# nuggy875/NeRF_pytorch_paeng

Measured on AMD Instinct MI355X. Metric: rays/sec (4096-ray batch, 64c+128f samples) + 800×800 frame render ms, higher is better.
Workload: dtype f32

## Files before the change

### nerf_pytorch_paeng_amd/csrc/api.hip

```cpp
#include <string>
#include "half_layout.h"

namespace minerf {

ABI_ERROR_STATE(, MI_NERF_EHIP)

int device_cus() {
    static std::atomic<int> cus[MN_MAX_DEVICES] = {};
    int dev = 0;
    if (hipGetDevice(&dev) != hipSuccess) return 256;
    std::atomic<int>& slot = cus[dev & (MN_MAX_DEVICES - 1)];
    int c = slot.load(std::memory_order_relaxed);
    if (c <= 0) {
        hipDeviceProp_t prop;
        c = (hipGetDeviceProperties(&prop, dev) == hipSuccess && prop.multiProcessorCount > 0) ? prop.multiProcessorCount : 256;
        slot.store(c, std::memory_order_relaxed);
    }
    return c;
}
int ensure_lds_opt_in(LdsOptIn& state, const void* kernel) {
    int dev = 0;
    MN_HIP(hipGetDevice(&dev));
    std::atomic<bool>& done = state.done[dev & (MN_MAX_DEVICES - 1)];
    if (!done.load(std::memory_order_acquire)) {
        MN_HIP(hipFuncSetAttribute(kernel, hipFuncAttributeMaxDynamicSharedMemorySize, 160 * 1024));
        done.store(true, std::memory_order_release);
    }
    return MI_NERF_OK;
}

int mlp_rays_fp32(const mi_nerf_net*, const void*, const float*, const float*, int64_t, int, float*, hipStream_t);
int mlp_embedded_fp32(const mi_nerf_net*, const void*, const float*, int64_t, float*, hipStream_t);
int mlp_rays_bf16(const mi_nerf_net*, const void*, const float*, const float*, int64_t, int, float*, hipStream_t, int points_per_wave, const StratDraw* strat,
                  FineDraw* fine = nullptr);
int mlp_rays_f16(const mi_nerf_net*, const void*, const float*, const float*, int64_t, int, float*, hipStream_t, int points_per_wave, const StratDraw* strat,
                 FineDraw* fine);
int mlp_rays_f16s(const mi_nerf_net*, const void*, const float*, const float*, int64_t, int, float*, hipStream_t);
int mlp_rays_f16s_stash(const mi_nerf_net*, const void*, const float*, const float*, int64_t, int, float*, float*, float*, float*, unsigned*, unsigned*,
                        hipStream_t);
int wgrad_products(int, const float* const*, const int*, const int*, const float* const*, const int*, const int*, int64_t, float* const*, const int*,
                   float* const*, void*, size_t, hipStream_t, bool);
int mlp_rays_fp32_stash(const mi_nerf_net*, const void*, const float*, const float*, int64_t, int, float*, float*, float*, float*, unsigned*,
                        unsigned*, hipStream_t);
int mlp_backward_fp32(const mi_nerf_net*, const void*, const void*, const float*, const float*, int64_t, int, const float*, const void*, void*,
                      size_t, float*, int, hipStream_t, const float*, int64_t, int);
int mlp_embedded_fp32_stash(const mi_nerf_net*, const void*, const float*, int64_t, float*, float*, float*, float*, unsigned*, unsigned*,
                            hipStream_t);
int train_layout(const mi_nerf_net*, int64_t, int, mi_nerf_train_layout*);
size_t wgrad_scratch_bytes();
int pack_apply(const int32_t*, const float*, size_t, void*, hipStream_t);
int frames_image_metrics(const float*, const float*, int64_t, float*, void*, size_t, hipStream_t);
int frames_nanmax(const float*, int64_t, float*, void*, size_t, hipStream_t);
int frames_to8b(const float*, int64_t, const float*, unsigned char*, hipStream_t);
int frames_rays_rgb(int, int, const float*, const float*, const float*, int64_t, float*, hipStream_t);
// ... 326 lines not shown
    return frames_rays_rgb(W, H, k4, poses, images, n_img, out, (hipStream_t)st);
}
int mi_nerf_permute_rows(const float* src, const int64_t* perm, int64_t n, int row_floats, float* dst, void* st) {
    return frames_permute_rows(src, perm, n, row_floats, dst, (hipStream_t)st);
}

size_t mi_nerf_render_workspace_bytes(const mi_nerf_render_cfg* cfg, int64_t n_rays) {
    mi_nerf_workspace_layout L;
    if (workspace_layout(cfg, n_rays, &L)) return 0;
    return L.total;
}
int mi_nerf_render_workspace_layout(const mi_nerf_render_cfg* cfg, int64_t n_rays, mi_nerf_workspace_layout* out) {
    return workspace_layout(cfg, n_rays, out);
}

int mi_nerf_render_rays(const mi_nerf_net* net, const void* packed_c, const void* packed_f, const mi_nerf_render_cfg* cfg,
                        const float* rays, int64_t n, const float* t_rand, const float* u, void* ws, size_t ws_bytes,
                        float* rgb_c, float* disp_c, float* rgb_f, float* disp_f, void* stream) {
    hipStream_t st = (hipStream_t)stream;
    mi_nerf_workspace_layout L;
    if (int rc = workspace_layout(cfg, n, &L)) return rc;
    if (n == 0) return MI_NERF_OK;
    MN_CHECK_ARG(ws_bytes >= L.total, "workspace too small: %zu < %zu", ws_bytes, L.total);
    MN_CHECK_ARG(rays && rgb_c && disp_c && packed_c && (ws || L.total == 0), "NULL pointer");
    MN_CHECK_ARG(cfg->Nf == 0 || (packed_f && rgb_f && disp_f), "fine pass needs packed_fine and outputs");
    MN_CHECK_ARG(cfg->reserved == 0, "mi_nerf_render_cfg.reserved must be 0");
    char* w = (char*)ws;
    float* z_c = (float*)(w + L.z_c);
    float* raw_c = (float*)(w + L.raw_c);
    float* wts_c = (float*)(w + L.weights_c);
    const int Sc = cfg->Sc, St = cfg->Sc + cfg->Nf;
    ModePlan p;
    if (int rc = mode_plan(cfg->mode, &p)) return rc;
    if (p.coarse == Family::F16 || p.fine == Family::F16)
        if (int rc = check_net_half(net, "f16")) return rc;
    if (p.coarse == Family::F16S || p.fine == Family::F16S)
        if (int rc = check_net_f16s_forward(net)) return rc;
    FineDraw fd{};
    if (p.coarse == Family::BF16 || p.coarse == Family::F16) {
        const StratDraw sd{cfg->near_, cfg->far_, t_rand, cfg->seed, cfg->ray_offset, z_c};
        if (cfg->Nf > 0) fd = FineDraw{cfg->Nf, cfg->det, u, cfg->seed, cfg->ray_offset, rgb_c, disp_c, wts_c, (float*)(w + L.z_f), false};
        if (int rc = mlp_rays_family(p.coarse, net, packed_c, rays, nullptr, n, Sc, raw_c, st, p.points_per_wave, &sd,
                                     cfg->Nf > 0 && p.points_per_wave == 0 ? &fd : nullptr))
            return rc;
    } else {
        if (int rc = stage_stratified(n, Sc, cfg->near_, cfg->far_, t_rand, cfg->seed, cfg->ray_offset, z_c, st)) return rc;
        if (int rc = mlp_rays_family(p.coarse, net, packed_c, rays, z_c, n, Sc, raw_c, st, p.points_per_wave)) return rc;
    }
    if (cfg->Nf == 0) return stage_composite(raw_c, z_c, rays, 6, n, Sc, rgb_c, disp_c, nullptr, wts_c, nullptr, st);
    {
        float* z_f = (float*)(w + L.z_f);
        float* raw_f = (float*)(w + L.raw_f);
        if (!fd.taken)
            if (int rc = stage_composite_fine_z(raw_c, z_c, rays, n, Sc, cfg->Nf, cfg->det, u, cfg->seed, cfg->ray_offset, rgb_c, disp_c, wts_c, z_f, st))
                return rc;
        if (int rc = mlp_rays_family(p.fine, net, packed_f, rays, z_f, n, St, raw_f, st, p.points_per_wave)) return rc;
        if (int rc = stage_composite(raw_f, z_f, rays, 6, n, St, rgb_f, disp_f, nullptr, nullptr, nullptr, st)) return rc;
    }
    return MI_NERF_OK;
}

int mi_nerf_time_mlp_rays(const mi_nerf_net* net, const void* packed, const float* rays, const float* z, int64_t n_rays, int S,
                          float* raw, int iters, int mode, float* avg_ms, void* stream) {
    hipStream_t st = (hipStream_t)stream;
    MN_CHECK_ARG(iters >= 1 && avg_ms, "bad iters / NULL output");
    ModePlan p;
    if (int rc = mode_plan(mode, &p)) return rc;
    MN_CHECK_ARG(p.coarse == p.fine, "MI_NERF_MODE_* %d is two kernel families (mi_nerf_render_rays only): one network, one kernel family", mode);
    if (p.fine == Family::F16)
        if (int rc = check_net_half(net, "f16")) return rc;
// ... 86 lines not shown
```

### nerf_pytorch_paeng_amd/csrc/layout.h

```cpp
#pragma once
#include <stdint.h>
#include <stddef.h>

namespace minerf {

constexpr int QUAD_BYTES = 1024;
constexpr int SLOT_QUADS = 16;
constexpr int SLOT_BYTES = QUAD_BYTES * SLOT_QUADS;
constexpr int HEADER_BYTES = 1024;
constexpr uint32_t BLOB_MAGIC = 0x4D494E46u;

__host__ __device__ constexpr int pe_ksteps(int L) { return ((3 * L + 2 + 3) / 4) * 4; }

constexpr int KERNEL_LX = 10, KERNEL_LD = 4;

constexpr int MAX_KERNEL_WIDTH = 512;
__host__ __device__ constexpr int kernel_width(int W) { return W <= 128 ? 128 : (W <= 256 ? 256 : (W <= 384 ? 384 : 512)); }
__host__ __device__ constexpr bool wide_kernel_width(int Wk) { return Wk > 256; }
__host__ __device__ constexpr int pe_ksteps16(int L) { return (((3 * L + 1) / 2 + 1 + 3) / 4) * 4; }
__host__ __device__ constexpr bool native_width(int W) { return W == 128 || W == 256; }

struct BlobLayout {
    uint32_t stream_off;
    uint32_t stream_bytes_hoist;
// ... 24 lines not shown
    uint32_t quads = pe_quads;
    for (int l = 1; l < D; ++l) quads += h_quads + ((skip >= 0 && l == skip + 1) ? pe_quads : 0);
    quads += h_quads;
    quads += (uint32_t)(W / 2 / 4) * (NT / 2);
    b.stream_off = HEADER_BYTES;
    b.stream_bytes_hoist = round_up_u32(quads, SLOT_QUADS) * QUAD_BYTES;
    uint32_t full = round_up_u32(quads, SLOT_QUADS) + round_up_u32((uint32_t)(pe_ksteps(L_d) / 4) * (NT / 2), SLOT_QUADS);
    b.stream_bytes_full = full * QUAD_BYTES;
    b.side_off = b.stream_off + b.stream_bytes_full;
    uint32_t f = 0;
    b.bias_trunk = f; f += (uint32_t)D * W;
    b.bias_feat = f;  f += W;
    b.bias_d = f;     f += W / 2;
    b.dens_w = f;     f += W;
    b.dens_b = f;     f += 4;
    b.color_w = f;    f += 3 * (W / 2);
    b.color_b = f;    f += 4;
    b.wdir_t = f;     f += (uint32_t)in_d * (W / 2);
    b.side_floats = round_up_u32(f, 4);
    b.total_bytes = b.side_off + b.side_floats * 4;
    return b;
}

struct SideTables {
    const char* stream;
    const float* side;
    int D;
    int skip_layer;
    unsigned stream_bytes;
    unsigned side_floats;
    unsigned o_bias_trunk, o_bias_feat, o_bias_d, o_wdir_t;
    unsigned o_dens_w, o_dens_b, o_color_w, o_color_b;
    unsigned o_head_b;
};
inline int skip_layer_of(int D, int skip) { return (skip >= 0 && skip + 1 < D) ? skip + 1 : -1; }

inline SideTables side_tables(const BlobLayout& L, const void* packed_dev, int D, int skip, bool full_stream) {
    SideTables t{};
    t.stream = (const char*)packed_dev + L.stream_off;
    t.side = (const float*)((const char*)packed_dev + L.side_off);
    t.D = D;
    t.skip_layer = skip_layer_of(D, skip);
    t.stream_bytes = full_stream ? L.stream_bytes_full : L.stream_bytes_hoist;
    t.side_floats = L.side_floats;
    t.o_bias_trunk = L.bias_trunk; t.o_bias_feat = L.bias_feat; t.o_bias_d = L.bias_d; t.o_wdir_t = L.wdir_t;
    t.o_dens_w = L.dens_w; t.o_dens_b = L.dens_b; t.o_color_w = L.color_w; t.o_color_b = L.color_b;
// ... 39 lines not shown
```

### nerf_pytorch_paeng_amd/csrc/mlp_fp32.hip

```cpp
#include <stdlib.h>
#include <vector>
#include "common.h"
#include "layout.h"
#include "mlp_core.h"


namespace minerf {


template <int L, bool SLOW, int NPE>
__device__ __forceinline__ void encode_regs(float (&pe)[NPE], const float (&p)[3], int hh) {
#pragma unroll
    for (int s = 0; s < 3 * L; ++s) {
        const float y = p[s % 3] * (float)(1 << (s / 3));
        pe[s] = SLOW ? sin_cos_slow(y, hh) : sin_cos_fast(y, hh);
    }
    pe[3 * L] = hh ? p[1] : p[0];
    pe[3 * L + 1] = hh ? 0.0f : p[2];
#pragma unroll
    for (int s = 3 * L + 2; s < NPE; ++s) pe[s] = 0.0f;
}

template <int L, int NPE>
__device__ __forceinline__ void gather_regs(float (&pe)[NPE], const float* row, int hh, bool valid, int L_net) {
// ... 158 lines not shown
            }
        }
        MN_STAMP(4);
        const float* cw = side + a.o_color_w;
        const float r0 = xhalf_sum(dot_half<HN / 2>(h2, cw, hh)) + side[a.o_color_b + 0];
        const float r1 = xhalf_sum(dot_half<HN / 2>(h2, cw + W / 2, hh)) + side[a.o_color_b + 1];
        const float r2 = xhalf_sum(dot_half<HN / 2>(h2, cw + W, hh)) + side[a.o_color_b + 2];
        if (valid && hh == 0) {
            f32x4 o; o[0] = r0; o[1] = r1; o[2] = r2; o[3] = dens;
            *(f32x4*)(a.out + out_idx * 4) = o;
        }
        MN_STAMP(5);
    }
#ifdef MN_DIAG
    if (a.diag && lane == 0) {
        unsigned long long* d = a.diag + ((size_t)blockIdx.x * 4 + wave) * 8;
        for (int i = 0; i < 8; ++i) d[i] = seg[i];
    }
#endif
    asm volatile("s_waitcnt vmcnt(0)" ::: "memory");
    __syncthreads();
}

static int check_net(const mi_nerf_net* net) {
    MN_CHECK_ARG(net != nullptr, "net is NULL");
    MN_CHECK_ARG(net->W >= 2 && net->W <= MAX_KERNEL_WIDTH, "unsupported width W=%d (the fp32 inference kernels run 2 <= W <= %d, padded to 128 / 256 / 384 / 512)", net->W, MAX_KERNEL_WIDTH);
    MN_CHECK_ARG(net->D >= 2 && net->D <= 16, "unsupported depth D=%d", net->D);
    MN_CHECK_ARG(net->L_x >= 0 && net->L_x <= KERNEL_LX && net->L_d >= 0 && net->L_d <= KERNEL_LD,
                 "unsupported encoding L_x=%d L_d=%d (the kernels evaluate up to %d / %d frequencies)", net->L_x, net->L_d, KERNEL_LX, KERNEL_LD);
    MN_CHECK_ARG(net->skip >= -1, "bad skip=%d", net->skip);
    return MI_NERF_OK;
}

int mlp_rays_fp32_wide(const mi_nerf_net*, const void*, const float*, const float*, int64_t, int, float*, hipStream_t);
int mlp_embedded_fp32_wide(const mi_nerf_net*, const void*, const float*, int64_t, float*, hipStream_t);

template <int W, int MODE, bool STASH = false>
static int launch(const MlpArgs& args_in, hipStream_t st) {
    MlpArgs args = args_in;
    auto kern = mlp_fp32_kernel<W, MODE, 10, 4, STASH>;
    static LdsOptIn opt_in = {};
    size_t lds;
    int grid;
    if (int rc = plan_launch<W, MODE>(args, (const void*)kern, opt_in, lds, grid)) return rc;
#ifdef MN_DIAG
    {
        MlpArgs da = args;
        unsigned long long* dbuf = nullptr;
        const size_t n = (size_t)grid * 4 * 8 + 16 * 512;
        MN_HIP(hipMalloc(&dbuf, n * 8));
        MN_HIP(hipMemsetAsync(dbuf, 0, n * 8, st));
        da.diag = dbuf;
        hipLaunchKernelGGL(kern, dim3(grid), dim3(256), lds, st, da);
        MN_HIP(hipStreamSynchronize(st));
        std::vector<unsigned long long> hbuf(n);
        MN_HIP(hipMemcpy(hbuf.data(), dbuf, n * 8, hipMemcpyDeviceToHost));
        (void)hipFree(dbuf);
        const double tiles = (double)((args.n_wtiles + 4 * grid - 1) / (4 * grid));
        static const char* names[6] = {"prologue", "layer0", "trunk", "dens+feature", "viewdir", "colour+store"};
        double tot = 0;
        fprintf(stderr, "[mn_diag] W=%d MODE=%d grid=%d tiles/wg=%.1f  cycles per tile (mean over waves):\n", W, MODE, grid, tiles);
        for (int sgi = 0; sgi < 6; ++sgi) {
            double sum = 0;
            for (size_t w = 0; w < (size_t)grid * 4; ++w) sum += (double)hbuf[w * 8 + sgi];
            const double per = sum / ((double)grid * 4) / tiles;
            tot += per;
            fprintf(stderr, "[mn_diag]   %-14s %10.0f\n", names[sgi], per);
        }
        fprintf(stderr, "[mn_diag]   %-14s %10.0f\n", "total", tot);
        if (const char* e = getenv("MN_DIAG_KQ")) {
            const int wsel = atoi(e);
            const unsigned long long* lg = hbuf.data() + (size_t)grid * 32 + (size_t)wsel * 512;
            fprintf(stderr, "[mn_diag] k-quad deltas (cycles; ideal %d) of wave %d, tile 2:", 4 * 64 * (W / 32), wsel);
            for (int i = 1; i < 500 && lg[i]; ++i) fprintf(stderr, "%s%llu", (i % 16 == 1) ? "\n[mn_diag]   " : " ", lg[i] - lg[i - 1]);
            fprintf(stderr, "\n");
        }
        return MI_NERF_OK;
    }
#endif
    hipLaunchKernelGGL(kern, dim3(grid), dim3(256), lds, st, args);
    MN_LAUNCH_CHECK("mlp_fp32_kernel");
    return MI_NERF_OK;
}

int mlp_rays_fp32(const mi_nerf_net* net, const void* packed_dev, const float* rays_dev, const float* z_dev,
                  int64_t n_rays, int S, float* raw_dev, hipStream_t st) {
    if (int rc = check_net(net)) return rc;
    MN_CHECK_ARG(n_rays >= 0 && S >= 1, "bad sizes n_rays=%lld S=%d", (long long)n_rays, S);
    if (n_rays == 0) return MI_NERF_OK;
    MN_CHECK_ARG(packed_dev && rays_dev && z_dev && raw_dev, "NULL device pointer");
    if (wide_kernel_width(kernel_width(net->W))) return mlp_rays_fp32_wide(net, packed_dev, rays_dev, z_dev, n_rays, S, raw_dev, st);
    MlpArgs a{};
    fill_common(a, net, packed_dev, false);
    fill_rays<32>(a, rays_dev, z_dev, n_rays, S, raw_dev);
    return kernel_width(net->W) == 256 ? launch<256, 0>(a, st) : launch<128, 0>(a, st);
}

int mlp_rays_fp32_stash(const mi_nerf_net* net, const void* packed_dev, const float* rays_dev, const float* z_dev,
                        int64_t n_rays, int S, float* raw_dev, float* stash_h, float* stash_f, float* stash_g, unsigned* mask_h,
                        unsigned* mask_g, hipStream_t st) {
    if (int rc = check_net(net)) return rc;
    MN_CHECK_ARG(native_width(net->W), "the training kernels exist for W = 128 and 256 (got %d)", net->W);
    MN_CHECK_ARG(n_rays >= 0 && S >= 1, "bad sizes n_rays=%lld S=%d", (long long)n_rays, S);
    if (n_rays == 0) return MI_NERF_OK;
    MN_CHECK_ARG(packed_dev && rays_dev && z_dev && raw_dev && stash_h && stash_f && stash_g && mask_h && mask_g, "NULL device pointer");
    MlpArgs a{};
    fill_common(a, net, packed_dev, false);
    fill_rays<32>(a, rays_dev, z_dev, n_rays, S, raw_dev);
    a.stash_h = stash_h; a.stash_f = stash_f; a.stash_g = stash_g; a.stash_rows = (long long)n_rays * S;
    a.mask_h = mask_h; a.mask_g = mask_g;
    return net->W == 256 ? launch<256, 0, true>(a, st) : launch<128, 0, true>(a, st);
}

int mlp_embedded_fp32_stash(const mi_nerf_net* net, const void* packed_dev, const float* x_dev, int64_t n, float* out_dev, float* stash_h,
                            float* stash_f, float* stash_g, unsigned* mask_h, unsigned* mask_g, hipStream_t st) {
    if (int rc = check_net(net)) return rc;
    MN_CHECK_ARG(native_width(net->W), "the training kernels exist for W = 128 and 256 (got %d)", net->W);
    MN_CHECK_ARG(n >= 0, "bad n=%lld", (long long)n);
// ... 27 lines not shown
```

### nerf_pytorch_paeng_amd/dist.py

```python
from __future__ import annotations

import ctypes as C
from typing import Callable, Dict, Optional, Sequence, Tuple

import torch
import torch.distributed as dist

from ._lib import MiNerfError, check, dev_ptr, lib, stream_ptr

COMM_ID_BYTES = 128


def shard_rows(H: int, world: int, rank: int) -> Tuple[int, int]:
    base, extra = divmod(H, world)
    n = base + (1 if rank < extra else 0)
    row0 = rank * base + min(rank, extra)
    return row0, n


def shard_range(n: int, world: int, rank: int) -> Tuple[int, int]:
    return shard_rows(n, world, rank)


class TileComm:
# ... 127 lines not shown
        parts.append(out[r * max_rows * W:r * max_rows * W + nr * W])
    return torch.cat(parts, 0)


def assemble_tiles(tiles: Sequence[torch.Tensor], H: int, W: int) -> torch.Tensor:
    world = len(tiles)
    for r, t in enumerate(tiles):
        _, nr = shard_rows(H, world, r)
        if t.shape[0] != nr * W:
            raise ValueError(f"tile {r} of {world} has {t.shape[0]} rays, expected {nr * W}")
    return tiles[0] if world == 1 else torch.cat(list(tiles), 0)


def render_shard(H: int, W: int, K, pose, model, opts, world: int, rank: int, *, seed: int = 0, bf16: bool = False,
                 f16s: bool = False, coarse_f16s: bool = False) -> torch.Tensor:
    from . import nerf_process as NP
    from . import ops
    from .weights import packed_for
    packed = packed_for(model)
    r0, nr = shard_rows(H, world, rank)
    _, d = ops.make_o_d(W, H, K, pose, packed.device, row0=r0, n_rows=nr, want_origins=False)
    p = pose if isinstance(pose, torch.Tensor) else torch.as_tensor(pose)
    o = p[:3, -1].to(packed.device, torch.float32).expand(d.shape)
    rc, dc, rf, df = NP.batchify_rays_and_render_by_chunk(o, d, packed, None, H, W, K, opts, seed=seed, ray_offset=r0 * W, bf16=bf16, f16s=f16s,
                                                          coarse_f16s=coarse_f16s)
    rgb, disp = (rc, dc) if int(opts.N_samples_f) == 0 else (rf, df)
    return torch.cat([rgb, disp[:, None]], -1)


def render_frame(H: int, W: int, K, pose, model, opts, *, seed: int = 0, group=None, bf16: bool = False, f16s: bool = False,
                 render_rows_fn: Optional[Callable[[int, int], torch.Tensor]] = None, via: str = "torch",
                 force_collective: bool = False, coarse_f16s: bool = False) -> Tuple[torch.Tensor, torch.Tensor]:
    if dist.is_available() and dist.is_initialized():
        world, rank = dist.get_world_size(group), dist.get_rank(group)
    else:
        world, rank = 1, 0
    if render_rows_fn is None:
        local = render_shard(H, W, K, pose, model, opts, world, rank, seed=seed, bf16=bf16, f16s=f16s, coarse_f16s=coarse_f16s)
    else:
        local = render_rows_fn(*shard_rows(H, world, rank))
    full = gather_tiles(local, H, W, group, force_collective=force_collective, via=via)
    return full[:, :3].reshape(H, W, 3), full[:, 3].reshape(H, W)
```

### nerf_pytorch_paeng_amd/harness.py

```python
from __future__ import annotations

import os
import struct
import zlib
from typing import Dict, List, Optional, Sequence

import numpy as np
import torch

from . import nerf_process as NP
from . import ops
from ._lib import MiNerfError, as_f32_dev
from .rays import make_o_d


def write_png(path: str, img: np.ndarray) -> None:
    a = np.ascontiguousarray(img)
    if a.dtype != np.uint8:
        raise MiNerfError(f"write_png wants uint8, got {a.dtype}")
    if a.ndim == 3 and a.shape[2] == 1:
        a = a[:, :, 0]
    if a.ndim == 2:
        color, raw = 0, a
    elif a.ndim == 3 and a.shape[2] == 3:
# ... 141 lines not shown
    grid = getattr(opts, "baked", None)
    if grid is not None:
        return grid.device
    view = getattr(opts, "mesh_view", None)
    if view is not None:
        return view.verts.device
    return next(model.parameters()).device if isinstance(model, torch.nn.Module) else model.device


def _render_pose(model, posenc, K, pose, hw, opts):
    img_h, img_w = hw
    view = getattr(opts, "mesh_view", None)
    if view is not None:
        from .mesh import Camera
        frame = view.render(Camera(img_h, img_w, K, pose[:3, :4]), near=float(getattr(opts, "mesh_view_near", 1e-3)),
                            cull=int(getattr(opts, "mesh_view_cull", 0)), bg=getattr(opts, "mesh_view_bg", (1.0, 1.0, 1.0)))
        return frame.rgb.reshape(-1, 3), frame.disp.reshape(-1)
    rays_o, rays_d = make_o_d(img_w, img_h, K, pose[:3, :4])
    grid = getattr(opts, "baked", None)
    if grid is not None:
        rays = torch.cat([rays_o.reshape(-1, 3), rays_d.reshape(-1, 3)], -1)
        rgb, disp, _, _ = grid.render(rays, step=getattr(opts, "baked_step", None), T_min=float(getattr(opts, "baked_T_min", 0.0) or 0.0))
        return rgb, disp
    rgb_c, disp_c, rgb_f, disp_f = NP.batchify_rays_and_render_by_chunk(rays_o, rays_d, model, posenc, img_h, img_w, K, opts, **_precision(opts),
                                                                        occupancy=getattr(opts, "occupancy", None))
    return (rgb_c, disp_c) if int(opts.N_samples_f) == 0 else (rgb_f, disp_f)


def test(idx, i_test, posenc, model, test_imgs, gt_intrinsic, gt_extrinsic, hw, opts, *, log_dir: Optional[str] = None,
         save_dir: Optional[str] = None, keep_frames: bool = False, ssim: bool = False, lpips=None) -> Dict:
    want_ssim = bool(ssim) or bool(getattr(opts, "ssim", False))
    lpips_model = lpips if lpips is not None else getattr(opts, "lpips", None)
    want_lpips = lpips_model is not None
    col_lpips = 3 if want_ssim else 2
    if isinstance(model, torch.nn.Module):
        model.eval()
        if log_dir is not None:
            load_checkpoint(_ckpt_path(log_dir, opts.exp_name, idx), model)
    if save_dir is not None:
        os.makedirs(save_dir, exist_ok=True)
    img_h, img_w = hw
    dev = _device_of(model, opts)
    n_pose = len(gt_extrinsic)
    want_frames = save_dir is not None or keep_frames
    metrics = torch.empty(n_pose, col_lpips + int(want_lpips), dtype=torch.float32, device=dev)
    rgbs8 = torch.empty(n_pose, img_h, img_w, 3, dtype=torch.uint8, device=dev) if want_frames else None
    disps8 = torch.empty(n_pose, img_h, img_w, 1, dtype=torch.uint8, device=dev) if want_frames else None
    with torch.no_grad():
# ... 240 lines not shown
```

### nerf_pytorch_paeng_amd/nerf_process.py

```python
from __future__ import annotations

from typing import Dict, Optional

import torch

from . import ops
from ._lib import MiNerfError, as_f32_dev
from .weights import PackedNeRF, packed_for
from . import train_path
from . import occupancy as occ
from . import occupancy_train
from . import geometry as geo

MAX_RAYS_PER_LAUNCH = 1 << 20

_rng = {"seed": 0, "calls": 0}


def manual_seed(seed: int) -> None:
    _rng["seed"], _rng["calls"] = int(seed), 0


def _next_seed(seed: Optional[int]) -> int:
    if seed is not None:
# ... 70 lines not shown
        return geo.composite_geo_backward(raw, z, d, 0.0, 1.0, g_rgb, g_acc, g_depth, None, g_wts), None, None, None


def post_process(outputs, z_vals, rays_d, *, weights_grad: bool = False):
    z = as_f32_dev(z_vals)
    raw = as_f32_dev(outputs, z.device)
    d = as_f32_dev(rays_d, z.device)
    if torch.is_grad_enabled() and raw.requires_grad:
        return _Composite.apply(raw, z.detach(), d.detach(), bool(weights_grad))
    return ops.composite(raw, z, d, want_all=True)


raw2outputs = post_process


def run_network(model, embedded, is_fine: bool = False):
    if train_path.wants_grad(model):
        return model(embedded, is_fine)
    packed = packed_for(model)
    return ops.mlp_embedded(packed.net, packed.blob(is_fine), as_f32_dev(embedded, packed.device))


def _render(rays: torch.Tensor, packed: PackedNeRF, opts, t_rand, u, seed: int, ray_offset: int, prec: ops.Precision,
            intermediates: bool, occupancy=None, geometry: bool = False) -> Dict[str, torch.Tensor]:
    n = rays.shape[0]
    dev = rays.device
    Sc, Nf = int(opts.N_samples_c), int(opts.N_samples_f)
    det = _det(opts)
    cfg = ops.render_cfg(float(opts.near), float(opts.far), Sc, Nf, det, seed=seed, ray_offset=ray_offset)
    cfg.mode = prec.mode
    if t_rand is not None:
        t_rand = as_f32_dev(t_rand, dev)
    elif intermediates:
        t_rand = ops.fill_uniform(seed, 0, ray_offset, n, Sc, dev)
    if Nf > 0 and not det:
        if u is not None:
            u = as_f32_dev(u, dev)
        elif intermediates:
            u = ops.fill_uniform(seed, 1, ray_offset, n, Nf, dev)
    else:
        u = None
    net, blob_c, blob_f = packed.kernel_blobs(prec)
    stats = None
    if occupancy is None:
        rgb_c, disp_c, rgb_f, disp_f, ws = ops.render_rays(net, blob_c, blob_f if Nf > 0 else None, cfg, rays, t_rand, u)
        views = ops.workspace_views
    else:
        rgb_c, disp_c, rgb_f, disp_f, ws, stats = occ.render_rays(net, blob_c, blob_f if Nf > 0 else None, cfg, occupancy, rays, t_rand, u)
        occupancy.last_stats = occ.add_stats(occupancy.last_stats, stats)
        views = occ.workspace_views
    out = {"rgb_c": rgb_c, "disp_c": disp_c}
    if Nf > 0:
        out["rgb_f"], out["disp_f"] = rgb_f, disp_f
    if geometry:
        v = views(cfg, n, ws)
        for key in ("c", "f") if Nf > 0 else ("c",):
            extra = geo.composite_geo(v["raw_" + key], v["z_" + key], rays, float(opts.near), float(opts.far))
            out.update({name + "_" + key: t for name, t in zip(geo.EXTRA_KEYS, (extra[2], extra[4], extra[5]))})
    if intermediates:
        for k, v in views(cfg, n, ws).items():
            out["_" + k] = v
        out["_t_rand"], out["_u"] = t_rand, u
        if stats is not None:
            out["_occ_stats"] = stats
    return out


def _occupancy_arg(occupancy, training: bool, prec: ops.Precision):
    if occupancy is None:
        return None
    if training:
        raise MiNerfError("occupancy= is an inference feature (call under torch.no_grad(), or freeze the model); to train with a grid pass it as "
                          "train_occupancy=")
    if not isinstance(occupancy, occ.OccupancyGrid):
        raise MiNerfError(f"occupancy must be an occupancy.OccupancyGrid, got {type(occupancy).__name__}")
    occ.check_precision(prec)
    occupancy.last_stats = None
    return occupancy


def _train_occupancy_arg(grid, training: bool, prec: ops.Precision):
    if grid is None:
        return None
    if not isinstance(grid, occ.OccupancyGrid):
        raise MiNerfError(f"train_occupancy must be an occupancy.OccupancyGrid, got {type(grid).__name__}")
    if not training:
        raise MiNerfError("train_occupancy= is a training feature: gradients are disabled or no parameter of the model requires them "
                          "(under torch.no_grad() render with occupancy=)")
    if prec.coarse != prec.fine or prec.fine not in ("fp32", "f16s"):
        raise MiNerfError(f"training with a grid runs fp32 or f16s for both networks (got coarse {prec.coarse}, fine {prec.fine})")
    grid.last_stats = None
    return grid


def _train_f16s(prec: ops.Precision, intermediates: bool = False) -> bool:
    if prec.fine not in ("fp32", "f16s") or intermediates:
        raise MiNerfError("the training path has no bf16 / f16 mode (fp32, or f16s=True: split-precision forward, fp32 backward) and returns no intermediates")
    return prec.fine == "f16s"


def _geometry_kw(geometry, ray_grad=False) -> Dict[str, bool]:
    return {**({"geometry": True} if geometry else {}), **({"ray_grad": True} if ray_grad else {})}


def _ray_grad_arg(ray_grad, train_occupancy) -> bool:
    if ray_grad and train_occupancy is not None:
        raise MiNerfError("ray_grad=True with train_occupancy= is not built: the occupancy-training node differentiates the parameters only")
    return bool(ray_grad)


def render_rays(rays, model, posenc, opts, *, t_rand=None, u=None, seed=None, ray_offset: int = 0, bf16: bool = False,
                return_intermediates: bool = False, f16s: bool = False, coarse_f16s: bool = False, f16: bool = False, coarse_f16: bool = False,
                occupancy=None, train_occupancy=None, geometry: bool = False, ray_grad: bool = False):
    prec = ops.precision(bf16, f16s, coarse_f16s, f16, coarse_f16)
    ray_grad = _ray_grad_arg(ray_grad, train_occupancy)
    training = train_path.wants_grad(model) or train_path.wants_ray_grad(model, ray_grad, rays)
    occupancy = _occupancy_arg(occupancy, training, prec)
    train_occupancy = _train_occupancy_arg(train_occupancy, training, prec)
    if training:
        train_f16s = _train_f16s(prec, return_intermediates)
        if rays.dim() != 2 or rays.shape[1] != 6:
            raise MiNerfError(f"rays must be [n, 6] (o, d), got {tuple(rays.shape)}")
        if train_occupancy is not None:
            return occupancy_train.render_train(rays, model, opts, train_occupancy, t_rand=t_rand, u=u, seed=_next_seed(seed),
                                                ray_offset=int(ray_offset), f16s=train_f16s, **_geometry_kw(geometry))
        return train_path.render_train(rays, model, opts, t_rand=t_rand, u=u, seed=_next_seed(seed), ray_offset=int(ray_offset), f16s=train_f16s,
                                       **_geometry_kw(geometry, ray_grad))
    packed = packed_for(model)
    rays = as_f32_dev(rays, packed.device)
    if rays.dim() != 2 or rays.shape[1] != 6:
        raise MiNerfError(f"rays must be [n, 6] (o, d), got {tuple(rays.shape)}")
    if occupancy is not None and rays.shape[0] > occ.MAX_RAYS_PER_LAUNCH:
        raise MiNerfError(f"render_rays with a grid takes at most {occ.MAX_RAYS_PER_LAUNCH} rays per call (batchify_rays_and_render_by_chunk slabs them)")
    return _render(rays, packed, opts, t_rand, u, _next_seed(seed), int(ray_offset), prec, return_intermediates, occupancy, **_geometry_kw(geometry))


def batchify_rays_and_render_by_chunk(ray_o, ray_d, model, posenc, H, W, K, opts, *, t_rand=None, u=None, seed=None,
                                      ray_offset: int = 0, bf16: bool = False, f16s: bool = False, coarse_f16s: bool = False, f16: bool = False,
                                      coarse_f16: bool = False, occupancy=None, train_occupancy=None, geometry: bool = False,
                                      ray_grad: bool = False):
    prec = ops.precision(bf16, f16s, coarse_f16s, f16, coarse_f16)
    ray_grad = _ray_grad_arg(ray_grad, train_occupancy)
    training = train_path.wants_grad(model) or train_path.wants_ray_grad(model, ray_grad, ray_o, ray_d)
    occupancy = _occupancy_arg(occupancy, training, prec)
    train_occupancy = _train_occupancy_arg(train_occupancy, training, prec)
    train_f16s = _train_f16s(prec) if training else False
    packed = None if training else packed_for(model)
    dev = next(model.parameters()).device if training else packed.device
    ray_d = as_f32_dev(ray_d, dev)
    flat_d = ray_d.reshape(-1, 3)
    ray_o = ray_o.to(dev) if ray_o.device != dev else ray_o
    flat_o = ray_o.to(torch.float32).expand(ray_d.shape).reshape(-1, 3)
    if getattr(opts, "data_type", None) == "llff":
        k00 = K[0][0]
        focal = float(k00.item()) if isinstance(k00, torch.Tensor) else float(k00)
        if ray_grad:
            from . import pose
            flat_o, flat_d = pose.ndc_rays(H, W, focal, 1.0, flat_o, flat_d)
        else:
            flat_o, flat_d = ndc_rays(H, W, focal, 1.0, flat_o, flat_d)
    rays = torch.cat((flat_o, flat_d), dim=-1)
    N = rays.shape[0]
    seed = _next_seed(seed)
    Nf = int(opts.N_samples_f)
    parts = []
    train_stats = None
    slab = train_path.MAX_TRAIN_RAYS if training else (MAX_RAYS_PER_LAUNCH if occupancy is None else occ.MAX_RAYS_PER_LAUNCH)
    for i in range(0, N, slab):
        j = min(N, i + slab)
        tr, uu = (None if t_rand is None else t_rand[i:j]), (None if u is None else u[i:j])
        if train_occupancy is not None:
            parts.append(occupancy_train.render_train(rays[i:j].contiguous(), model, opts, train_occupancy, t_rand=tr, u=uu, seed=seed,
                                                      ray_offset=int(ray_offset) + i, f16s=train_f16s, **_geometry_kw(geometry)))
            train_stats = occ.add_stats(train_stats, train_occupancy.last_stats)
        elif training:
            parts.append(train_path.render_train(rays[i:j].contiguous(), model, opts, t_rand=tr, u=uu, seed=seed,
                                                 ray_offset=int(ray_offset) + i, f16s=train_f16s, **_geometry_kw(geometry, ray_grad)))
        else:
            parts.append(_render(rays[i:j], packed, opts, tr, uu, seed, int(ray_offset) + i, prec, False, occupancy, **_geometry_kw(geometry)))
    if train_occupancy is not None:
        train_occupancy.last_stats = train_stats
    def cat(key):
        return parts[0][key] if len(parts) == 1 else torch.cat([p[key] for p in parts], dim=0)
    res = (cat("rgb_c"), cat("disp_c"), cat("rgb_f"), cat("disp_f")) if Nf > 0 else (cat("rgb_c"), cat("disp_c"), None, None)
    if geometry:
        return (*res, {name + "_" + key: cat(name + "_" + key) for key in (("c", "f") if Nf > 0 else ("c",)) for name in geo.EXTRA_KEYS})
    return res
```

### nerf_pytorch_paeng_amd/ops.py

```python
from __future__ import annotations

import ctypes as C
from typing import Dict, NamedTuple, Optional, Sequence, Tuple

import numpy as np
import torch

from . import _lib as L
from ._lib import MiNerfError, Net, RenderCfg, TrainLayout, WorkspaceLayout, check, dev_ptr, lib, stream_ptr


def _guard(device):
    device = torch.device(device)
    if device.type != "cuda":
        raise MiNerfError(f"tensors must live on a HIP device (got {device}); this path has no CPU fallback")
    return torch.cuda.device(device)


def make_net(D: int, W: int, skip: int = 4, L_x: int = 10, L_d: int = 4) -> Net:
    return Net(D, W, skip, L_x, L_d)


F16S_FWD_MAX_D = 14
F16S_DGRAD_MAX_D = 15
# ... 594 lines not shown
    if on not in _FAMILIES:
        raise MiNerfError(f"no precision mode sets {' + '.join(on)}: none (fp32), bf16, f16s, f16, or bf16 with one of coarse_f16s / coarse_f16")
    coarse, fine = _FAMILIES[on]
    p = Precision(coarse, fine, 0 if fine in ("fp32", "f16s") else int(points_per_wave))
    if p not in _MODES:
        raise MiNerfError(f"points_per_wave={points_per_wave}: 0 (chosen per launch), or 64 / 32 with bf16 alone")
    return p


def render_cfg(near: float, far: float, Sc: int, Nf: int, det: bool, bf16: bool = False, points_per_wave: int = 0, seed: int = 0,
               ray_offset: int = 0, f16s: bool = False, coarse_f16s: bool = False, f16: bool = False, coarse_f16: bool = False) -> RenderCfg:
    mode = precision(bf16, f16s, coarse_f16s, f16, coarse_f16, points_per_wave).mode
    return RenderCfg(float(near), float(far), int(Sc), int(Nf), int(bool(det)), mode, int(seed) & 0xFFFFFFFF, 0, int(ray_offset))


def workspace_layout(cfg: RenderCfg, n: int) -> WorkspaceLayout:
    wl = WorkspaceLayout()
    check(lib().mi_nerf_render_workspace_layout(C.byref(cfg), n, C.byref(wl)), "mi_nerf_render_workspace_layout")
    return wl


def render_rays(net: Net, packed_c: torch.Tensor, packed_f: Optional[torch.Tensor], cfg: RenderCfg, rays: torch.Tensor,
                t_rand: Optional[torch.Tensor], u: Optional[torch.Tensor], workspace: Optional[torch.Tensor] = None,
                out: Optional[Sequence[torch.Tensor]] = None):
    n = rays.shape[0]
    dev = rays.device
    if tuple(rays.shape) != (n, 6) or (t_rand is not None and tuple(t_rand.shape) != (n, cfg.Sc)):
        raise MiNerfError(f"rays [n,6] / t_rand [n,{cfg.Sc}] expected, got {tuple(rays.shape)} / {None if t_rand is None else tuple(t_rand.shape)}")
    if cfg.Nf > 0 and not cfg.det and u is not None and tuple(u.shape) != (n, cfg.Nf):
        raise MiNerfError(f"u [n,{cfg.Nf}] expected")
    wl = workspace_layout(cfg, n)
    if workspace is None or workspace.numel() < wl.total:
        workspace = torch.empty(max(wl.total, 256), dtype=torch.uint8, device=dev)
    if out is None:
        rgb_c = torch.empty(n, 3, dtype=torch.float32, device=dev)
        disp_c = torch.empty(n, dtype=torch.float32, device=dev)
        rgb_f = torch.empty(n, 3, dtype=torch.float32, device=dev) if cfg.Nf > 0 else None
        disp_f = torch.empty(n, dtype=torch.float32, device=dev) if cfg.Nf > 0 else None
    else:
        rgb_c, disp_c, rgb_f, disp_f = out
    with _guard(dev):
        check(lib().mi_nerf_render_rays(C.byref(net), dev_ptr(packed_c, "packed_coarse", torch.uint8, 16),
                                        dev_ptr(packed_f, "packed_fine", torch.uint8, 16), C.byref(cfg), dev_ptr(rays, "rays"), n,
                                        dev_ptr(t_rand, "t_rand"), dev_ptr(u, "u") if (cfg.Nf > 0 and not cfg.det) else None,
                                        dev_ptr(workspace, "workspace", torch.uint8, 256), workspace.numel(), dev_ptr(rgb_c), dev_ptr(disp_c),
                                        dev_ptr(rgb_f), dev_ptr(disp_f), stream_ptr(dev)), "mi_nerf_render_rays")
    return rgb_c, disp_c, rgb_f, disp_f, workspace


def workspace_views(cfg: RenderCfg, n: int, workspace: torch.Tensor) -> Dict[str, torch.Tensor]:
    wl = workspace_layout(cfg, n)
    Sc, St = cfg.Sc, cfg.Sc + cfg.Nf
    def view(off, shape):
        cnt = int(np.prod(shape))
        return workspace[off:off + cnt * 4].view(torch.float32).view(*shape)
    v = {"z_c": view(wl.z_c, (n, Sc)), "raw_c": view(wl.raw_c, (n, Sc, 4)), "weights_c": view(wl.weights_c, (n, Sc))}
    if cfg.Nf > 0:
        v["z_f"] = view(wl.z_f, (n, St))
        v["raw_f"] = view(wl.raw_f, (n, St, 4))
    return v


def time_mlp_rays(net: Net, packed: torch.Tensor, rays: torch.Tensor, z: torch.Tensor, raw: torch.Tensor, iters: int, bf16: bool = False,
# ... 16 lines not shown
```

Before: 490,500.

## Add density-only coarse MLP kernel when the coarse image is not needed

Adds a coarse_image=False mode in which the coarse pass runs a new fp32 kernel that evaluates only the trunk and density head, skipping the direction encoding and the view-dependent RGB layers. The weight stream is truncated to the trunk bytes, and the coarse rgb/disp outputs are written into scratch workspace. The frame render and distributed paths opt into this mode when a fine pass exists. This cuts coarse-pass MLP FLOPs and weight traffic. The risk is that the coarse RGB written as zeros could affect fine sampling if compositing weights depended on it; they depend only on density.

Result: no change. 490,300, median of 2 (-0.0%).

```diff
diff --git a/nerf_pytorch_paeng_amd/csrc/api.hip b/nerf_pytorch_paeng_amd/csrc/api.hip
--- a/nerf_pytorch_paeng_amd/csrc/api.hip
+++ b/nerf_pytorch_paeng_amd/csrc/api.hip
@@ -30,6 +30,7 @@
 }
 
 int mlp_rays_fp32(const mi_nerf_net*, const void*, const float*, const float*, int64_t, int, float*, hipStream_t);
+int mlp_rays_fp32_density(const mi_nerf_net*, const void*, const float*, const float*, int64_t, int, float*, hipStream_t);
 int mlp_embedded_fp32(const mi_nerf_net*, const void*, const float*, int64_t, float*, hipStream_t);
 int mlp_rays_bf16(const mi_nerf_net*, const void*, const float*, const float*, int64_t, int, float*, hipStream_t, int points_per_wave, const StratDraw* strat,
                   FineDraw* fine = nullptr);
@@ -402,10 +403,16 @@
     if (int rc = workspace_layout(cfg, n, &L)) return rc;
     if (n == 0) return MI_NERF_OK;
     MN_CHECK_ARG(ws_bytes >= L.total, "workspace too small: %zu < %zu", ws_bytes, L.total);
-    MN_CHECK_ARG(rays && rgb_c && disp_c && packed_c && (ws || L.total == 0), "NULL pointer");
+    const bool coarse_image = rgb_c != nullptr || disp_c != nullptr;
+    MN_CHECK_ARG(rays && (rgb_c || cfg->Nf > 0) && (disp_c || cfg->Nf > 0) && packed_c && (ws || L.total == 0), "NULL pointer");
+    MN_CHECK_ARG((rgb_c != nullptr) == (disp_c != nullptr), "rgb_c and disp_c go together: both, or both NULL (fine image only)");
     MN_CHECK_ARG(cfg->Nf == 0 || (packed_f && rgb_f && disp_f), "fine pass needs packed_fine and outputs");
     MN_CHECK_ARG(cfg->reserved == 0, "mi_nerf_render_cfg.reserved must be 0");
     char* w = (char*)ws;
+    if (!coarse_image) {
+        rgb_c = (float*)(w + L.raw_f);
+        disp_c = rgb_c + 3 * (size_t)n;
+    }
     float* z_c = (float*)(w + L.z_c);
     float* raw_c = (float*)(w + L.raw_c);
     float* wts_c = (float*)(w + L.weights_c);
@@ -425,7 +432,9 @@
             return rc;
     } else {
         if (int rc = stage_stratified(n, Sc, cfg->near_, cfg->far_, t_rand, cfg->seed, cfg->ray_offset, z_c, st)) return rc;
-        if (int rc = mlp_rays_family(p.coarse, net, packed_c, rays, z_c, n, Sc, raw_c, st, p.points_per_wave)) return rc;
+        if (!coarse_image && p.coarse == Family::FP32) {
+            if (int rc = mlp_rays_fp32_density(net, packed_c, rays, z_c, n, Sc, raw_c, st)) return rc;
+        } else if (int rc = mlp_rays_family(p.coarse, net, packed_c, rays, z_c, n, Sc, raw_c, st, p.points_per_wave)) return rc;
     }
     if (cfg->Nf == 0) return stage_composite(raw_c, z_c, rays, 6, n, Sc, rgb_c, disp_c, nullptr, wts_c, nullptr, st);
     {
diff --git a/nerf_pytorch_paeng_amd/csrc/layout.h b/nerf_pytorch_paeng_amd/csrc/layout.h
--- a/nerf_pytorch_paeng_amd/csrc/layout.h
+++ b/nerf_pytorch_paeng_amd/csrc/layout.h
@@ -70,6 +70,15 @@
     return b;
 }
 
+inline uint32_t trunk_stream_bytes(int D, int W_net, int skip) {
+    const int W = kernel_width(W_net), NT = W / 32;
+    const uint32_t pe_quads = (uint32_t)(pe_ksteps(KERNEL_LX) / 4) * NT;
+    const uint32_t h_quads = (uint32_t)(W / 2 / 4) * NT;
+    uint32_t quads = round_up_u32(pe_quads, SLOT_QUADS);
+    for (int l = 1; l < D; ++l) quads += round_up_u32(h_quads, SLOT_QUADS) + ((skip >= 0 && l == skip + 1) ? round_up_u32(pe_quads, SLOT_QUADS) : 0);
+    return quads * QUAD_BYTES;
+}
+
 struct SideTables {
     const char* stream;
     const float* side;
diff --git a/nerf_pytorch_paeng_amd/csrc/mlp_fp32.hip b/nerf_pytorch_paeng_amd/csrc/mlp_fp32.hip
--- a/nerf_pytorch_paeng_amd/csrc/mlp_fp32.hip
+++ b/nerf_pytorch_paeng_amd/csrc/mlp_fp32.hip
@@ -204,6 +204,70 @@
     __syncthreads();
 }
 
+template <int W, int LX>
+__global__ __launch_bounds__(256) __attribute__((amdgpu_waves_per_eu(1, 1)))
+void mlp_fp32_density_kernel(const MlpArgs a) {
+    constexpr int NT = W / 32;
+    constexpr int HN = W / 2;
+    constexpr int KPE = pe_ksteps(LX);
+    constexpr int AL = 4;
+    extern __shared__ __attribute__((aligned(16))) char smem[];
+    float* side = (float*)(smem + RING_BYTES);
+    const int tid = threadIdx.x;
+    const int lane = tid & 63;
+    const int wave = __builtin_amdgcn_readfirstlane(tid >> 6);
+    const int col = lane & 31, hh = lane >> 5;
+
+    for (unsigned i = tid * 4; i < a.side_floats; i += 256 * 4) *(f32x4*)(side + i) = *(const f32x4*)(a.side + i);
+
+    const long long n_wg_tiles = (a.n_wtiles + 3) >> 2;
+    if ((long long)blockIdx.x >= n_wg_tiles) return;
+
+    WRing ring = ring_start(a.stream, a.stream_bytes, smem, wave, lane);
+
+    f32x16 acc[8];
+    f32x4 aq[8];
+    float h[HN];
+    float pe[KPE];
+    ring_advance(ring);
+#pragma unroll
+    for (int t = 0; t < NT; ++t) aq[t] = ring_read(smem, ring, lane, t);
+
+    RayTileWalk<32> walk = {};
+    walk.start(a, (long long)blockIdx.x * 4 + wave, col);
+    for (long long it = 0; it < a.n_iter; ++it) {
+        const bool wave_active = walk.active(a);
+        const long long ray = walk.ray(a);
+        const int sample = walk.chunk(a) * 32 + col;
+        const bool valid = wave_active && sample < a.S;
+        const long long out_idx = ray * a.S + (sample < a.S ? sample : a.S - 1);
+        const float o[3] = {walk.o[0], walk.o[1], walk.o[2]}, d[3] = {walk.d[0], walk.d[1], walk.d[2]};
+        const float zv = walk.z;
+        walk.advance(a, col);
+        float p[3];
+        sample_point(p, o, d, zv);
+        if (__builtin_expect(point_is_fast<LX>(p), 1)) encode_regs<LX, false>(pe, p, hh);
+        else encode_regs<LX, true>(pe, p, hh);
+        acc_init<NT>(acc, side + a.o_bias_trunk, hh);
+        gemm_part<NT, KPE, NT, AL>(acc, pe, aq, smem, ring, lane);
+#pragma unroll 1
+        for (int l = 1; l < a.D; ++l) {
+            acc_to_b<NT, true>(acc, h);
+            acc_init<NT>(acc, side + a.o_bias_trunk + l * W, hh);
+            if (l == a.skip_layer) gemm_part<NT, KPE, NT, AL>(acc, pe, aq, smem, ring, lane);
+            gemm_part<NT, HN, NT, AL>(acc, h, aq, smem, ring, lane);
+        }
+        acc_to_b<NT, true>(acc, h);
+        const float dens = xhalf_sum(dot_half<HN>(h, side + a.o_dens_w, hh)) + side[a.o_dens_b];
+        if (valid && hh == 0) {
+            f32x4 o4; o4[0] = 0.0f; o4[1] = 0.0f; o4[2] = 0.0f; o4[3] = dens;
+            *(f32x4*)(a.out + out_idx * 4) = o4;
+        }
+    }
+    asm volatile("s_waitcnt vmcnt(0)" ::: "memory");
+    __syncthreads();
+}
+
 static int check_net(const mi_nerf_net* net) {
     MN_CHECK_ARG(net != nullptr, "net is NULL");
     MN_CHECK_ARG(net->W >= 2 && net->W <= MAX_KERNEL_WIDTH, "unsupported width W=%d (the fp32 inference kernels run 2 <= W <= %d, padded to 128 / 256 / 384 / 512)", net->W, MAX_KERNEL_WIDTH);
@@ -217,10 +281,16 @@
 int mlp_rays_fp32_wide(const mi_nerf_net*, const void*, const float*, const float*, int64_t, int, float*, hipStream_t);
 int mlp_embedded_fp32_wide(const mi_nerf_net*, const void*, const float*, int64_t, float*, hipStream_t);
 
-template <int W, int MODE, bool STASH = false>
+template <int W, int MODE, bool STASH, bool DENS>
+static auto kernel_entry() {
+    if constexpr (DENS) return &mlp_fp32_density_kernel<W, 10>;
+    else return &mlp_fp32_kernel<W, MODE, 10, 4, STASH>;
+}
+
+template <int W, int MODE, bool STASH = false, bool DENS = false>
 static int launch(const MlpArgs& args_in, hipStream_t st) {
     MlpArgs args = args_in;
-    auto kern = mlp_fp32_kernel<W, MODE, 10, 4, STASH>;
+    auto kern = kernel_entry<W, MODE, STASH, DENS>();
     static LdsOptIn opt_in = {};
     size_t lds;
     int grid;
@@ -261,7 +331,8 @@
     }
 #endif
     hipLaunchKernelGGL(kern, dim3(grid), dim3(256), lds, st, args);
-    MN_LAUNCH_CHECK("mlp_fp32_kernel");
+    if constexpr (DENS) MN_LAUNCH_CHECK("mlp_fp32_density_kernel");
+    else MN_LAUNCH_CHECK("mlp_fp32_kernel");
     return MI_NERF_OK;
 }
 
@@ -276,6 +347,20 @@
     fill_common(a, net, packed_dev, false);
     fill_rays<32>(a, rays_dev, z_dev, n_rays, S, raw_dev);
     return kernel_width(net->W) == 256 ? launch<256, 0>(a, st) : launch<128, 0>(a, st);
+}
+
+int mlp_rays_fp32_density(const mi_nerf_net* net, const void* packed_dev, const float* rays_dev, const float* z_dev,
+                          int64_t n_rays, int S, float* raw_dev, hipStream_t st) {
+    if (int rc = check_net(net)) return rc;
+    MN_CHECK_ARG(n_rays >= 0 && S >= 1, "bad sizes n_rays=%lld S=%d", (long long)n_rays, S);
+    if (n_rays == 0) return MI_NERF_OK;
+    MN_CHECK_ARG(packed_dev && rays_dev && z_dev && raw_dev, "NULL device pointer");
+    if (wide_kernel_width(kernel_width(net->W))) return mlp_rays_fp32_wide(net, packed_dev, rays_dev, z_dev, n_rays, S, raw_dev, st);
+    MlpArgs a{};
+    fill_common(a, net, packed_dev, false);
+    a.stream_bytes = trunk_stream_bytes(net->D, net->W, net->skip);
+    fill_rays<32>(a, rays_dev, z_dev, n_rays, S, raw_dev);
+    return kernel_width(net->W) == 256 ? launch<256, 0, false, true>(a, st) : launch<128, 0, false, true>(a, st);
 }
 
 int mlp_rays_fp32_stash(const mi_nerf_net* net, const void* packed_dev, const float* rays_dev, const float* z_dev,
diff --git a/nerf_pytorch_paeng_amd/dist.py b/nerf_pytorch_paeng_amd/dist.py
--- a/nerf_pytorch_paeng_amd/dist.py
+++ b/nerf_pytorch_paeng_amd/dist.py
@@ -173,9 +173,10 @@
     _, d = ops.make_o_d(W, H, K, pose, packed.device, row0=r0, n_rows=nr, want_origins=False)
     p = pose if isinstance(pose, torch.Tensor) else torch.as_tensor(pose)
     o = p[:3, -1].to(packed.device, torch.float32).expand(d.shape)
+    fine = int(opts.N_samples_f) > 0
     rc, dc, rf, df = NP.batchify_rays_and_render_by_chunk(o, d, packed, None, H, W, K, opts, seed=seed, ray_offset=r0 * W, bf16=bf16, f16s=f16s,
-                                                          coarse_f16s=coarse_f16s)
-    rgb, disp = (rc, dc) if int(opts.N_samples_f) == 0 else (rf, df)
+                                                          coarse_f16s=coarse_f16s, **({"coarse_image": False} if fine else {}))
+    rgb, disp = (rf, df) if fine else (rc, dc)
     return torch.cat([rgb, disp[:, None]], -1)
 
 
diff --git a/nerf_pytorch_paeng_amd/harness.py b/nerf_pytorch_paeng_amd/harness.py
--- a/nerf_pytorch_paeng_amd/harness.py
+++ b/nerf_pytorch_paeng_amd/harness.py
@@ -187,8 +187,10 @@
         rays = torch.cat([rays_o.reshape(-1, 3), rays_d.reshape(-1, 3)], -1)
         rgb, disp, _, _ = grid.render(rays, step=getattr(opts, "baked_step", None), T_min=float(getattr(opts, "baked_T_min", 0.0) or 0.0))
         return rgb, disp
+    occupancy = getattr(opts, "occupancy", None)
+    fine_only = int(opts.N_samples_f) > 0 and occupancy is None
     rgb_c, disp_c, rgb_f, disp_f = NP.batchify_rays_and_render_by_chunk(rays_o, rays_d, model, posenc, img_h, img_w, K, opts, **_precision(opts),
-                                                                        occupancy=getattr(opts, "occupancy", None))
+                                                                        occupancy=occupancy, **({"coarse_image": False} if fine_only else {}))
     return (rgb_c, disp_c) if int(opts.N_samples_f) == 0 else (rgb_f, disp_f)
 
 
diff --git a/nerf_pytorch_paeng_amd/nerf_process.py b/nerf_pytorch_paeng_amd/nerf_process.py
--- a/nerf_pytorch_paeng_amd/nerf_process.py
+++ b/nerf_pytorch_paeng_amd/nerf_process.py
@@ -116,7 +116,7 @@
 
 
 def _render(rays: torch.Tensor, packed: PackedNeRF, opts, t_rand, u, seed: int, ray_offset: int, prec: ops.Precision,
-            intermediates: bool, occupancy=None, geometry: bool = False) -> Dict[str, torch.Tensor]:
+            intermediates: bool, occupancy=None, geometry: bool = False, coarse_image: bool = True) -> Dict[str, torch.Tensor]:
     n = rays.shape[0]
     dev = rays.device
     Sc, Nf = int(opts.N_samples_c), int(opts.N_samples_f)
@@ -137,7 +137,8 @@
     net, blob_c, blob_f = packed.kernel_blobs(prec)
     stats = None
     if occupancy is None:
-        rgb_c, disp_c, rgb_f, disp_f, ws = ops.render_rays(net, blob_c, blob_f if Nf > 0 else None, cfg, rays, t_rand, u)
+        rgb_c, disp_c, rgb_f, disp_f, ws = ops.render_rays(net, blob_c, blob_f if Nf > 0 else None, cfg, rays, t_rand, u,
+                                                           **({} if coarse_image else {"coarse_image": False}))
         views = ops.workspace_views
     else:
         rgb_c, disp_c, rgb_f, disp_f, ws, stats = occ.render_rays(net, blob_c, blob_f if Nf > 0 else None, cfg, occupancy, rays, t_rand, u)
@@ -160,6 +161,16 @@
     return out
 
 
+def _fine_only_arg(opts, training: bool = False, intermediates: bool = False, occupancy=None, train_occupancy=None, geometry: bool = False,
+                   ray_grad: bool = False) -> None:
+    bad = [name for name, on in (("N_samples_f == 0 (the coarse image is the only output)", int(opts.N_samples_f) <= 0),
+                                 ("gradients enabled (the training path returns both images)", training), ("ray_grad=True", ray_grad),
+                                 ("return_intermediates=True", intermediates), ("occupancy=", occupancy is not None),
+                                 ("train_occupancy=", train_occupancy is not None), ("geometry=True", geometry)) if on]
+    if bad:
+        raise MiNerfError("coarse_image=False does not go with " + ", ".join(bad))
+
+
 def _occupancy_arg(occupancy, training: bool, prec: ops.Precision):
     if occupancy is None:
         return None
@@ -205,10 +216,12 @@
 
 def render_rays(rays, model, posenc, opts, *, t_rand=None, u=None, seed=None, ray_offset: int = 0, bf16: bool = False,
                 return_intermediates: bool = False, f16s: bool = False, coarse_f16s: bool = False, f16: bool = False, coarse_f16: bool = False,
-                occupancy=None, train_occupancy=None, geometry: bool = False, ray_grad: bool = False):
+                occupancy=None, train_occupancy=None, geometry: bool = False, ray_grad: bool = False, coarse_image: bool = True):
     prec = ops.precision(bf16, f16s, coarse_f16s, f16, coarse_f16)
     ray_grad = _ray_grad_arg(ray_grad, train_occupancy)
     training = train_path.wants_grad(model) or train_path.wants_ray_grad(model, ray_grad, rays)
+    if not coarse_image:
+        _fine_only_arg(opts, training, return_intermediates, occupancy, train_occupancy, geometry, ray_grad)
     occupancy = _occupancy_arg(occupancy, training, prec)
     train_occupancy = _train_occupancy_arg(train_occupancy, training, prec)
     if training:
@@ -226,16 +239,19 @@
         raise MiNerfError(f"rays must be [n, 6] (o, d), got {tuple(rays.shape)}")
     if occupancy is not None and rays.shape[0] > occ.MAX_RAYS_PER_LAUNCH:
         raise MiNerfError(f"render_rays with a grid takes at most {occ.MAX_RAYS_PER_LAUNCH} rays per call (batchify_rays_and_render_by_chunk slabs them)")
-    return _render(rays, packed, opts, t_rand, u, _next_seed(seed), int(ray_offset), prec, return_intermediates, occupancy, **_geometry_kw(geometry))
+    return _render(rays, packed, opts, t_rand, u, _next_seed(seed), int(ray_offset), prec, return_intermediates, occupancy, **_geometry_kw(geometry),
+                   **({} if coarse_image else {"coarse_image": False}))
 
 
 def batchify_rays_and_render_by_chunk(ray_o, ray_d, model, posenc, H, W, K, opts, *, t_rand=None, u=None, seed=None,
                                       ray_offset: int = 0, bf16: bool = False, f16s: bool = False, coarse_f16s: bool = False, f16: bool = False,
                                       coarse_f16: bool = False, occupancy=None, train_occupancy=None, geometry: bool = False,
-                                      ray_grad: bool = False):
+                                      ray_grad: bool = False, coarse_image: bool = True):
     prec = ops.precision(bf16, f16s, coarse_f16s, f16, coarse_f16)
     ray_grad = _ray_grad_arg(ray_grad, train_occupancy)
     training = train_path.wants_grad(model) or train_path.wants_ray_grad(model, ray_grad, ray_o, ray_d)
+    if not coarse_image:
+        _fine_only_arg(opts, training, False, occupancy, train_occupancy, geometry, ray_grad)
     occupancy = _occupancy_arg(occupancy, training, prec)
     train_occupancy = _train_occupancy_arg(train_occupancy, training, prec)
     train_f16s = _train_f16s(prec) if training else False
@@ -271,12 +287,16 @@
             parts.append(train_path.render_train(rays[i:j].contiguous(), model, opts, t_rand=tr, u=uu, seed=seed,
                                                  ray_offset=int(ray_offset) + i, f16s=train_f16s, **_geometry_kw(geometry, ray_grad)))
         else:
-            parts.append(_render(rays[i:j], packed, opts, tr, uu, seed, int(ray_offset) + i, prec, False, occupancy, **_geometry_kw(geometry)))
+            parts.append(_render(rays[i:j], packed, opts, tr, uu, seed, int(ray_offset) + i, prec, False, occupancy, **_geometry_kw(geometry),
+                                 **({} if coarse_image else {"coarse_image": False})))
     if train_occupancy is not None:
         train_occupancy.last_stats = train_stats
     def cat(key):
         return parts[0][key] if len(parts) == 1 else torch.cat([p[key] for p in parts], dim=0)
-    res = (cat("rgb_c"), cat("disp_c"), cat("rgb_f"), cat("disp_f")) if Nf > 0 else (cat("rgb_c"), cat("disp_c"), None, None)
+    if not coarse_image:
+        res = (None, None, cat("rgb_f"), cat("disp_f"))
+    else:
+        res = (cat("rgb_c"), cat("disp_c"), cat("rgb_f"), cat("disp_f")) if Nf > 0 else (cat("rgb_c"), cat("disp_c"), None, None)
     if geometry:
         return (*res, {name + "_" + key: cat(name + "_" + key) for key in (("c", "f") if Nf > 0 else ("c",)) for name in geo.EXTRA_KEYS})
     return res
diff --git a/nerf_pytorch_paeng_amd/ops.py b/nerf_pytorch_paeng_amd/ops.py
--- a/nerf_pytorch_paeng_amd/ops.py
+++ b/nerf_pytorch_paeng_amd/ops.py
@@ -640,9 +640,11 @@
 
 def render_rays(net: Net, packed_c: torch.Tensor, packed_f: Optional[torch.Tensor], cfg: RenderCfg, rays: torch.Tensor,
                 t_rand: Optional[torch.Tensor], u: Optional[torch.Tensor], workspace: Optional[torch.Tensor] = None,
-                out: Optional[Sequence[torch.Tensor]] = None):
+                out: Optional[Sequence[torch.Tensor]] = None, coarse_image: bool = True):
     n = rays.shape[0]
     dev = rays.device
+    if not coarse_image and cfg.Nf <= 0:
+        raise MiNerfError("coarse_image=False needs a fine pass (N_samples_f > 0): without one the coarse image is the only output")
     if tuple(rays.shape) != (n, 6) or (t_rand is not None and tuple(t_rand.shape) != (n, cfg.Sc)):
         raise MiNerfError(f"rays [n,6] / t_rand [n,{cfg.Sc}] expected, got {tuple(rays.shape)} / {None if t_rand is None else tuple(t_rand.shape)}")
     if cfg.Nf > 0 and not cfg.det and u is not None and tuple(u.shape) != (n, cfg.Nf):
@@ -651,12 +653,14 @@
     if workspace is None or workspace.numel() < wl.total:
         workspace = torch.empty(max(wl.total, 256), dtype=torch.uint8, device=dev)
     if out is None:
-        rgb_c = torch.empty(n, 3, dtype=torch.float32, device=dev)
-        disp_c = torch.empty(n, dtype=torch.float32, device=dev)
+        rgb_c = torch.empty(n, 3, dtype=torch.float32, device=dev) if coarse_image else None
+        disp_c = torch.empty(n, dtype=torch.float32, device=dev) if coarse_image else None
         rgb_f = torch.empty(n, 3, dtype=torch.float32, device=dev) if cfg.Nf > 0 else None
         disp_f = torch.empty(n, dtype=torch.float32, device=dev) if cfg.Nf > 0 else None
     else:
         rgb_c, disp_c, rgb_f, disp_f = out
+        if not coarse_image and (rgb_c is not None or disp_c is not None):
+            raise MiNerfError("coarse_image=False: out=(None, None, rgb_f, disp_f)")
     with _guard(dev):
         check(lib().mi_nerf_render_rays(C.byref(net), dev_ptr(packed_c, "packed_coarse", torch.uint8, 16),
                                         dev_ptr(packed_f, "packed_fine", torch.uint8, 16), C.byref(cfg), dev_ptr(rays, "rays"), n,
```
